# makezur/super_primitive

Measured on AMD Instinct MI355X. Metric: GN iters/sec (640x480x64-seg frame pairs), higher is better.
Workload: dtype f32; 1 GPU; Replica-shaped two-frame SfM, 640x480, 64 segments (grid, 4 px overlap), pyramid level 0 of a 3-level pyramid; BASELINE.json configs[1]; pairs_per_gpu=384, segment_pixels_per_pair=373056, optimiser=gn, tile_points=8192, span_points=4096, granule=64

## Files before the change

### super_primitive_amd/csrc/sp_cost.hip

```cpp
#include <type_traits>

#include "sp_solve_device.h"

namespace {

struct TileCtx {
    gptr_u32 pix;
    gptr_f4 src4;
    gptr_f32 trg;
    Cam Ks;
    Warp w;
    float shift;
    float gain, bias;
    float ax, ay;
    uint32_t row_bytes;
    int Wl, Hl;
    int start, count;
};

struct Geo {
    float qx, qy, qz;
    float zinv, zi;
    float px, py, pz;
};
// ... 293 lines not shown
                                           Pending& p) {
    const f32x2 colrow = rd_colrow(r, lane2);
    const float d = rd_depth(r, DT ? s.w * shift : fast_exp(s.w + shift));
    float x, y;
    backproject(colrow.x, colrow.y, d, c.Ks, ifx, ify, x, y);
    prepare_xyz(c, x, y, d, true, s.x, s.y, s.z, p);
}

__device__ __forceinline__ void prepare2_at(const PairConsts& k, f32x2 colrow, bool src_ok, float d, const f32x4 s, Pending2& p) {
    const f32x2 xy = pfma(colrow, k.ifxy, k.nKc) * d;
    const f32x2 qxy = pfma(k.R03, f32x2{xy.x, xy.x}, pfma(k.R14, f32x2{xy.y, xy.y}, pfma(k.R25, f32x2{d, d}, k.t01)));
    const float qz = fmaf(k.R6, xy.x, fmaf(k.R7, xy.y, fmaf(k.R8, d, k.t2)));
    const bool zguard = fabsf(qz) > 1e-6f;
    const float zinv = zguard ? __builtin_amdgcn_rcpf(qz) : 1e-6f;
    const f32x2 uv = qxy * k.Kf * zinv + k.Ktc;
    const f32x2 n = pfma(uv, k.invWH, f32x2{-1.f, -1.f});
    const bool ok = (fabsf(n.x) <= 0.99f) && (fabsf(n.y) <= 0.99f) && (qz > k.zmin) && src_ok && (d > 1e-7f);
    p.m = ok ? 1.f : 0.f;
    p.qxy = qxy; p.qz = qz;
    p.zinv = ok ? zinv : 0.f;
    p.zi = (ok && zguard) ? zinv : 0.f;
    p.srg = f32x2{s.x, s.y}; p.sb = s.z;
    const f32x2 ixy = pfma(n, k.sxy, k.sxy);
    const f32x2 fl{floorf(ixy.x), floorf(ixy.y)};
    p.wxy = ixy - fl;
    p.off0 = (uint32_t)fmaf(fl.y, k.row_bytes_f, fl.x * (float)(4u * SP_TEXEL_FLOATS));
}

struct Mix2 { f32x2 wa, wb, v; };
struct MixA { f32x2 ua, ub; };
struct AffAcc {
    float haa, hab, hbb, ba, bb;
    f32x2 pa01, pa[2], pb01, pb[2];
    float hda, hdb;
};

template <bool AFF = false>
__device__ __forceinline__ void finish_gn2(const PairConsts& k, const Pending2& p, const f32x3 a, const f32x3 b,
                                           const f32x3 cc, const f32x3 d, Mix2& o, float& cost_acc, float& n_acc,
                                           MixA* oa = nullptr, AffAcc* aa = nullptr) {
    const float eps = k.eps;
    const f32x2 a2{a.x, a.y}, b2{b.x, b.y}, c2{cc.x, cc.y}, d2{d.x, d.y};
    const f32x2 e3 = padd2(psub2(psub2(d2, c2), b2), a2);
    const f32x2 Er{b.x - a.x, cc.x - a.x}, Eg{b.y - a.y, cc.y - a.y}, Eb{b.z - a.z, cc.z - a.z};
    f32x2 e3b;
    e3b.x = (d.z - cc.z) - Eb.x;
    const f32x2 Gr = pfma_swz_lo(p.wxy, e3, Er), Gg = pfma_swz_hi(p.wxy, e3, Eg), Gb = pfma_swz_lo(p.wxy, e3b, Eb);
    const f32x2 it2{fmaf(p.wxy.y, Gr.y, fmaf(p.wxy.x, Er.x, a.x)), fmaf(p.wxy.y, Gg.y, fmaf(p.wxy.x, Eg.x, a.y))};
    const float itb = fmaf(p.wxy.y, Gb.y, fmaf(p.wxy.x, Eb.x, a.z));
    const f32x2 r2 = p.srg - pfma(k.gain, it2, k.bias2);
    const float rb = p.sb - fmaf(k.gain, itb, k.bias2.x);
    const float ar0 = fabsf(r2.x), ar1 = fabsf(r2.y), arb = fabsf(rb);
    auto absmax = [&](float r) { float m; asm("v_max_f32 %0, |%1|, %2" : "=v"(m) : "v"(r), "s"(eps)); return m; };
    const f32x2 wg2{__builtin_amdgcn_rcpf(absmax(r2.x)), __builtin_amdgcn_rcpf(absmax(r2.y))};
    const float wgb = __builtin_amdgcn_rcpf(absmax(rb));
    const f32x2 wGr = pmul_lo(wg2, Gr), wGg = pmul_hi(wg2, Gg), wGb = Gb * wgb;
    o.wa = pfma_lo(wGb, Gb, pfma_lo(wGg, Gg, pmul_lo(wGr, Gr)));
    o.wb = pfma_hi(wGb, Gb, pfma_hi(wGg, Gg, pmul_hi(wGr, Gr)));
    o.v = pfma(wGb, rb, pfma_hi(r2, wGg, pmul_lo(r2, wGr)));
    cost_acc = fmaf(p.m, (ar0 + ar1) + arb, cost_acc);
    n_acc += p.m;
    if constexpr (AFF) {
        const f32x2 ja2 = k.gain * it2;
        const float jab = k.gain * itb;
        const f32x2 wj2 = wg2 * ja2;
        const float wjb = wgb * jab;
        aa->haa = fmaf(p.m, fmaf(wjb, jab, wj2.x * ja2.x) + wj2.y * ja2.y, aa->haa);
        aa->hab = fmaf(-p.m, (wj2.x + wj2.y) + wjb, aa->hab);
        aa->hbb = fmaf(p.m, (wg2.x + wg2.y) + wgb, aa->hbb);
        aa->ba = fmaf(p.m, fmaf(wjb, rb, wj2.x * r2.x) + wj2.y * r2.y, aa->ba);
        aa->bb = fmaf(-p.m, fmaf(wgb, rb, wg2.x * r2.x) + wg2.y * r2.y, aa->bb);
        oa->ua = pfma(Gb, wjb, pfma_hi(wj2, Gg, pmul_lo(wj2, Gr)));
        oa->ub = (wGr + wGg) + wGb;
    }
}

struct GeoGn { f32x2 qxy; float qz, zinv, zi; };
template <bool AFF = false>
__device__ __forceinline__ void fold_gn2(const PairConsts& k, const GeoGn g, const Mix2 w, GnAcc& A, const MixA* wa = nullptr,
                                         AffAcc* aa = nullptr) {
    const f32x2 g2 = k.gab * g.zinv;
    const f32x2 Wa = w.wa * pmul_lo(g2, g2);
    const f32x2 Wb = w.wb * pmul_hi(g2, g2);
    const f32x2 V = -(w.v * g2);
    const f32x2 qxy = g.qxy;
    const f32x2 u = qxy * g.zi;
    const float ez = g.qz - k.t2;
    const f32x2 Q = pfma(-ez, u, qxy - k.t01);
    float nqy;
    asm("v_xor_b32 %0, 0x80000000, %1" : "=v"(nqy) : "v"(qxy.y));
    const f32x2 nA00{u.x, u.x * qxy.y}, A01{fmaf(u.x, qxy.x, g.qz), nqy};
    const f32x2 nA10{u.y, fmaf(u.y, qxy.y, g.qz)}, A11{u.y * qxy.x, qxy.x};
    const f32x2 nB00 = pfma_lo(Wa, nA00, pmul_hi(Wa, nA10)), B01 = pfma_lo(Wa, A01, pmul_hi(Wa, A11));
    const f32x2 nB10 = pfma_lo(Wb, nA00, pmul_hi(Wb, nA10)), B11 = pfma_lo(Wb, A01, pmul_hi(Wb, A11));
    const f32x2 P = pfma_lo(Q, Wa, pmul_hi(Q, Wb));
    A.h00 += Wa; A.h11 += Wb.y;
    A.h0[0] -= nB00; A.h0[1] += B01;
    A.h1[0] -= nB10; A.h1[1] += B11;
    A.blk[0] = pfma_lo(nA00, nB00, pfma_lo(nA10, nB10, A.blk[0]));
    A.blk[1] = pfnma_lo(nA00, B01, pfnma_lo(nA10, B11, A.blk[1]));
    A.blk[2] = pfma_hi(nA00, nB00, pfma_hi(nA10, nB10, A.blk[2]));
    A.blk[3] = pfnma_hi(nA00, B01, pfnma_hi(nA10, B11, A.blk[3]));
    A.blk[4] = pfma_lo(A01, B01, pfma_lo(A11, B11, A.blk[4]));
    A.blk[5] = pfma_hi(A01, B01, pfma_hi(A11, B11, A.blk[5]));
    A.bp01 += V;
    A.hd01 += P;
    A.bp[0] = pfnma_lo(V, nA00, pfnma_hi(V, nA10, A.bp[0]));
    A.bp[1] = pfma_lo(V, A01, pfma_hi(V, A11, A.bp[1]));
    A.hd[0] = pfnma_lo(P, nA00, pfnma_hi(P, nA10, A.hd[0]));
    A.hd[1] = pfma_lo(P, A01, pfma_hi(P, A11, A.hd[1]));
    A.D = pfma(Q, P, A.D);
    A.bd = pfma(Q, V, A.bd);
    if constexpr (AFF) {
        const f32x2 Ua = -(wa->ua * g2), Ub = wa->ub * g2;
        aa->pa01 += Ua;
        aa->pa[0] = pfnma_lo(Ua, nA00, pfnma_hi(Ua, nA10, aa->pa[0]));
        aa->pa[1] = pfma_lo(Ua, A01, pfma_hi(Ua, A11, aa->pa[1]));
        aa->hda = fmaf(Q.x, Ua.x, fmaf(Q.y, Ua.y, aa->hda));
        aa->pb01 += Ub;
        aa->pb[0] = pfnma_lo(Ub, nA00, pfnma_hi(Ub, nA10, aa->pb[0]));
        aa->pb[1] = pfma_lo(Ub, A01, pfma_hi(Ub, A11, aa->pb[1]));
        aa->hdb = fmaf(Q.x, Ub.x, fmaf(Q.y, Ub.y, aa->hdb));
    }
}

typedef const float __attribute__((address_space(4)))* cptr_f32;
struct ChunkRec { int pair, seg, start, count; };
typedef const ChunkRec __attribute__((address_space(4)))* cptr_i4;

struct SpanCursor {
    cptr_i4 chunks;
    cptr_f32 kld, kp_L;
    int q, q_end;
    int left;
    float shift;
    int nq_left;
    float nq_kld, nq_kpl;
};

template <int TRIP = SP_BLOCK>
__device__ __forceinline__ void cursor_fetch_next(SpanCursor& k) {
    if (k.q + 1 < k.q_end) {
        const int seg = k.chunks[k.q + 1].seg;
        k.nq_left = k.chunks[k.q + 1].count / TRIP;
        k.nq_kld = k.kld[seg];
        k.nq_kpl = k.kp_L[seg];
    }
}

template <bool DT>
__device__ __forceinline__ float cursor_shift(float kld, float kpl) { return DT ? fast_exp(kld - kpl) : kld - kpl; }

template <int TRIP = SP_BLOCK, bool DT = false>
__device__ __forceinline__ void cursor_init(SpanCursor& k, const SpPair& pr, const int4* chunks, int q0, int n) {
    k.chunks = (cptr_i4)chunks;
    k.kld = (cptr_f32)pr.kld;
    k.kp_L = (cptr_f32)pr.kp_L;
    k.q = q0; k.q_end = q0 + n;
    const int seg0 = k.chunks[q0].seg;
    k.left = k.chunks[q0].count / TRIP;
    k.shift = cursor_shift<DT>(k.kld[seg0], k.kp_L[seg0]);
    k.nq_left = 0; k.nq_kld = 0.f; k.nq_kpl = 0.f;
    cursor_fetch_next<TRIP>(k);
}

template <int TRIP = SP_BLOCK, bool DT = false>
__device__ __forceinline__ bool cursor_advance(SpanCursor& k, int& done_q) {
    done_q = k.q;
    if (--k.left > 0) return false;
    ++k.q;
    k.left = k.nq_left;
    k.shift = cursor_shift<DT>(k.nq_kld, k.nq_kpl);
    cursor_fetch_next<TRIP>(k);
    return true;
}

template <bool WT>
__device__ __forceinline__ void store_partial(float* p, float v) {
    if (WT) __hip_atomic_store(p, v, __ATOMIC_RELAXED, __HIP_MEMORY_SCOPE_AGENT);
    else *p = v;
}

__device__ __forceinline__ int lane_id() { return (int)__builtin_amdgcn_mbcnt_hi(~0u, __builtin_amdgcn_mbcnt_lo(~0u, 0u)); }

template <bool WT, bool AFF = false>
__device__ __forceinline__ void flush_segment_gn(GnAcc& A, float* __restrict__ rec, AffAcc* aa = nullptr) {
    const int lane = lane_id();
    int pos; bool ok;
    if constexpr (AFF) {
        float v[10] = {A.hd01.x, A.hd01.y, A.hd[0].x, A.hd[0].y, A.hd[1].x, A.hd[1].y, A.D.x + A.D.y, A.bd.x + A.bd.y, aa->hda, aa->hdb};
        wave_sum_to_lanes<10>(v, lane, pos, ok);
        if (ok) store_partial<WT>(rec + pos, v[0]);
        aa->hda = 0.f; aa->hdb = 0.f;
    } else {
        float v[10] = {A.hd01.x, A.hd01.y, A.hd[0].x, A.hd[0].y, A.hd[1].x, A.hd[1].y, A.D.x + A.D.y, A.bd.x + A.bd.y,
                       A.cost - A.cost_mark, A.n - A.n_mark};
        wave_sum_to_lanes<10>(v, lane, pos, ok);
        if (ok) store_partial<WT>(rec + pos, v[0]);
        A.cost_mark = A.cost; A.n_mark = A.n;
    }
    const f32x2 z{0.f, 0.f};
    A.hd01 = z; A.hd[0] = z; A.hd[1] = z; A.D = z; A.bd = z;
}

template <bool DT, bool WT, bool AFF = false, bool W64 = false, bool RD = false>
__device__ __forceinline__ void run_span_gn(const TileCtx& c, const SpPair& pr, const int4* __restrict__ chunks, int q0,
                                            int n_chunks, int total, float irls_eps, float* __restrict__ span_rec,
                                            float* __restrict__ seg_partials, float* lds, const SpRunDesc* rd = nullptr) {
    static_assert(!RD || (W64 && DT && !AFF), "run descriptors: wave spans on depth tables");
    constexpr int TRIP = W64 ? 64 : SP_BLOCK;
    constexpr int NV = AFF ? SP_GNA_PARTIAL_FLOATS : SP_GN_PARTIAL_FLOATS, NS = AFF ? SP_GNA_SEG_FLOATS : SP_GN_SEG_FLOATS;
    GnAcc A;
    AffAcc AA;
    MixA ma{f32x2{0.f, 0.f}, f32x2{0.f, 0.f}};
    {
        const f32x2 z{0.f, 0.f};
        AA.haa = AA.hab = AA.hbb = AA.ba = AA.bb = AA.hda = AA.hdb = 0.f;
        AA.pa01 = z; AA.pb01 = z; AA.pa[0] = z; AA.pa[1] = z; AA.pb[0] = z; AA.pb[1] = z;
    }
    {
        const f32x2 z{0.f, 0.f};
        A.h00 = z; A.bp01 = z; A.hd01 = z;
#pragma unroll
        for (int k = 0; k < 2; ++k) { A.h0[k] = z; A.h1[k] = z; A.bp[k] = z; A.hd[k] = z; }
#pragma unroll
        for (int k = 0; k < 6; ++k) A.blk[k] = z;
        A.D = z; A.bd = z;
        A.h11 = A.cost = A.n = A.cost_mark = A.n_mark = 0.f;
    }
    const int wave = __builtin_amdgcn_readfirstlane((int)(threadIdx.x >> 6));
    SpanCursor k;
    cursor_init<TRIP, DT>(k, pr, chunks, q0, n_chunks);
    const int start = k.chunks[q0].start;
    PairConsts kc;
    {
        const Warp& w = c.w;
        kc.ifxy = sgpr2(1.f / c.Ks.fx, 1.f / c.Ks.fy);
        kc.nKc = f32x2{-c.Ks.cx * (1.f / c.Ks.fx), -c.Ks.cy * (1.f / c.Ks.fy)};
        kc.R03 = sgpr2(w.R[0], w.R[3]);        kc.R14 = sgpr2(w.R[1], w.R[4]);      kc.R25 = sgpr2(w.R[2], w.R[5]);
        kc.t01 = f32x2{w.t[0], w.t[1]};        kc.Kf = sgpr2(w.Kt.fx, w.Kt.fy);     kc.Ktc = sgpr2(w.Kt.cx, w.Kt.cy);
        kc.invWH = sgpr2(2.f * w.invWm1, 2.f * w.invHm1);  kc.sxy = sgpr2(w.sx, w.sy);
        kc.gab = sgpr2(c.gain * c.ax * w.Kt.fx, c.gain * c.ay * w.Kt.fy);
        kc.bias2 = f32x2{c.bias, c.bias};      kc.eps2 = sgpr2(irls_eps, irls_eps);
        kc.R6 = sgpr(w.R[6]); kc.R7 = sgpr(w.R[7]); kc.R8 = sgpr(w.R[8]); kc.t2 = w.t[2];
        asm volatile("" : "+v"(kc.nKc), "+v"(kc.bias2), "+v"(kc.t01), "+v"(kc.t2));
        kc.gain = sgpr(c.gain); kc.bias = sgpr(c.bias); kc.zmin = sgpr(w.zmin); kc.eps = sgpr(irls_eps);
        kc.row_bytes_f = sgpr((float)(c.Wl * (int)(4u * SP_TEXEL_FLOATS)));
    }
    const rsrc_t r_pix = make_rsrc(c.pix + start, (uint32_t)total * 4u);
    const rsrc_t r_src = make_rsrc(c.src4 + start, (uint32_t)total * 16u);
    const rsrc_t r_trg = make_rsrc(c.trg, (uint32_t)c.Wl * (uint32_t)c.Hl * (4u * SP_TEXEL_FLOATS));
    const int n_iter = total / TRIP;
    uint32_t op = (W64 ? (threadIdx.x & 63u) : threadIdx.x) * 4u;
    constexpr int NT = 2;
    cptr_rd rg = (cptr_rd)rd + (start >> 6);
    f32x2 lane2{(float)(threadIdx.x & 63u), 0.f};
    if (RD) asm volatile("" : "+v"(lane2));
    struct Slot { Pending2 p; int q; bool last; };
    Slot S0, S1;
    {
        const f32x4 s = buf_load4<NT>(r_src, op * 4u);
        if (RD) prepare2_rd<DT>(kc, k.shift, rd_load(rg), lane2, s, S0.p);
        else {
            const uint32_t pw = (uint32_t)__builtin_amdgcn_raw_buffer_load_b32(r_pix, (int)op, 0, NT);
            prepare2<DT>(c, kc, k.shift, pw, s, S0.p);
        }
        S0.last = cursor_advance<TRIP, DT>(k, S0.q);
    }
    S1.p = S0.p;
    S1.p.zinv = 0.f; S1.p.zi = 0.f;
    S1.q = q0; S1.last = false;
    Mix2 m{f32x2{0.f, 0.f}, f32x2{0.f, 0.f}, f32x2{0.f, 0.f}};
    auto trip = [&](Slot& a, Slot& b) {
        op += 4u * TRIP;
        asm volatile("" : "+v"(op));
        const uint32_t pw = RD ? 0u : (uint32_t)__builtin_amdgcn_raw_buffer_load_b32(r_pix, (int)op, 0, NT);
        const f32x4 s = buf_load4<NT>(r_src, op * 4u);
        SpRunDesc rn;
        if (RD) { ++rg; rn = rd_load(rg); }
        f32x3 ta = buf_load3(r_trg, a.p.off0);
        f32x3 tb = buf_load3(r_trg, a.p.off0 + 4u * SP_TEXEL_FLOATS);
        f32x3 tc = buf_load3(r_trg, a.p.off0, c.row_bytes);
        f32x3 td = buf_load3(r_trg, a.p.off0 + 4u * SP_TEXEL_FLOATS, c.row_bytes);
        __builtin_amdgcn_sched_barrier(0);
        fold_gn2<AFF>(kc, GeoGn{b.p.qxy, b.p.qz, b.p.zinv, b.p.zi}, m, A, &ma, &AA);
        if (b.last) flush_segment_gn<WT, AFF>(A, seg_partials + (size_t)(W64 ? b.q : 4 * b.q + wave) * NS, &AA);
        __builtin_amdgcn_sched_barrier(0);
        asm volatile("" : "+v"(ta), "+v"(tb), "+v"(tc), "+v"(td), "+v"(A.blk[0]), "+v"(A.blk[1]), "+v"(A.blk[2]),
                     "+v"(A.blk[3]), "+v"(A.blk[4]), "+v"(A.blk[5]), "+v"(A.bp[0]), "+v"(A.bp[1]), "+v"(A.hd[0]),
                     "+v"(A.hd[1]), "+v"(A.D), "+v"(A.bd), "+v"(A.h00), "+v"(A.h0[0]), "+v"(A.h0[1]), "+v"(A.h1[0]), "+v"(A.h1[1]), "+v"(A.h11), "+v"(A.bp01), "+v"(A.hd01));
        finish_gn2<AFF>(kc, a.p, ta, tb, tc, td, m, A.cost, A.n, &ma, &AA);
        uint32_t pw_ = pw;
        f32x4 s_ = s;
        if (RD) asm volatile("" : "+v"(s_));
        else asm volatile("" : "+v"(pw_), "+v"(s_));
        if (RD) prepare2_rd<DT>(kc, k.shift, rn, lane2, s_, b.p);
        else prepare2<DT>(c, kc, k.shift, pw_, s_, b.p);
        b.last = cursor_advance<TRIP, DT>(k, b.q);
    };
    int j = 0;
    for (; j + 1 < n_iter; j += 2) { trip(S0, S1); trip(S1, S0); }
    if (j < n_iter) {
        trip(S0, S1);
        fold_gn2<AFF>(kc, GeoGn{S0.p.qxy, S0.p.qz, S0.p.zinv, S0.p.zi}, m, A, &ma, &AA);
        flush_segment_gn<WT, AFF>(A, seg_partials + (size_t)(W64 ? S0.q : 4 * S0.q + wave) * NS, &AA);
    } else {
        fold_gn2<AFF>(kc, GeoGn{S1.p.qxy, S1.p.qz, S1.p.zinv, S1.p.zi}, m, A, &ma, &AA);
        flush_segment_gn<WT, AFF>(A, seg_partials + (size_t)(W64 ? S1.q : 4 * S1.q + wave) * NS, &AA);
    }
    float acc[NV];
    acc[0] = A.cost;
    acc[1] = A.h00.x; acc[2] = A.h00.y;
    acc[3] = A.h0[0].x; acc[4] = A.h0[0].y; acc[5] = A.h0[1].x; acc[6] = A.h0[1].y;
    acc[7] = A.h11;
    acc[8] = A.h1[0].x; acc[9] = A.h1[0].y; acc[10] = A.h1[1].x; acc[11] = A.h1[1].y;
    acc[12] = A.blk[0].x; acc[13] = A.blk[0].y; acc[14] = A.blk[1].x; acc[15] = A.blk[1].y;
    acc[16] = A.blk[2].y; acc[17] = A.blk[3].x; acc[18] = A.blk[3].y;
    acc[19] = A.blk[4].x; acc[20] = A.blk[4].y; acc[21] = A.blk[5].y;
    acc[22] = A.bp01.x; acc[23] = A.bp01.y;
    acc[24] = A.bp[0].x; acc[25] = A.bp[0].y; acc[26] = A.bp[1].x; acc[27] = A.bp[1].y;
    acc[28] = A.n;
    if constexpr (AFF) {
        acc[29] = AA.haa; acc[30] = AA.hab; acc[31] = AA.hbb; acc[32] = AA.ba; acc[33] = AA.bb;
        acc[34] = AA.pa01.x; acc[35] = AA.pa01.y; acc[36] = AA.pa[0].x; acc[37] = AA.pa[0].y; acc[38] = AA.pa[1].x; acc[39] = AA.pa[1].y;
        acc[40] = AA.pb01.x; acc[41] = AA.pb01.y; acc[42] = AA.pb[0].x; acc[43] = AA.pb[0].y; acc[44] = AA.pb[1].x; acc[45] = AA.pb[1].y;
        acc[46] = acc[47] = 0.f;
    } else {
        acc[29] = acc[30] = acc[31] = 0.f;
    }
    if (W64) {
        int pos; bool ok;
        wave_sum_to_lanes<NV>(acc, (int)((op >> 2) & 63u), pos, ok);
        if (ok) store_partial<WT>(span_rec + pos, acc[0]);
    } else {
        const int tid = (int)((op >> 2) & (uint32_t)(SP_BLOCK - 1));
        const float tot = block_sum_to_thread<NV>(acc, lds, tid);
        if (tid < NV) store_partial<WT>(span_rec + tid, tot);
    }
}

template <bool DT, bool WT, bool W64 = false, bool RD = false>
__device__ __forceinline__ void run_span_grad(const TileCtx& c, const SpPair& pr, const int4* __restrict__ chunks, int q0,
                                              int n_chunks, int total, float* __restrict__ span_rec,
                                              float* __restrict__ seg_partials, float* lds, const SpRunDesc* rd = nullptr) {
    static_assert(!RD || (W64 && DT), "run descriptors: wave spans on depth tables");
    constexpr int TRIP = W64 ? 64 : SP_BLOCK;
    constexpr int NV = SP_GRAD_PARTIAL_FLOATS;
    float acc[NV];
#pragma unroll
    for (int i = 0; i < NV; ++i) acc[i] = 0.f;
    const int wave = __builtin_amdgcn_readfirstlane((int)(threadIdx.x >> 6));
    SpanCursor k;
    cursor_init<TRIP, DT>(k, pr, chunks, q0, n_chunks);
    const int start = k.chunks[q0].start;
    const float ifx = 1.f / c.Ks.fx, ify = 1.f / c.Ks.fy;
    const rsrc_t r_pix = make_rsrc(c.pix + start, (uint32_t)total * 4u);
    const rsrc_t r_src = make_rsrc(c.src4 + start, (uint32_t)total * 16u);
    const rsrc_t r_trg = make_rsrc(c.trg, (uint32_t)c.Wl * (uint32_t)c.Hl * (4u * SP_TEXEL_FLOATS));
    const int n_iter = total / TRIP;
    uint32_t op = (W64 ? (threadIdx.x & 63u) : threadIdx.x) * 4u;
    constexpr int NT = 2;
    cptr_rd rg = (cptr_rd)rd + (start >> 6);
    f32x2 lane2{(float)(threadIdx.x & 63u), 0.f};
    if (RD) asm volatile("" : "+v"(lane2));
    struct Slot { Pending p; int q; bool last; };
    Slot S0, S1;
    {
        const f32x4 s = buf_load4<NT>(r_src, op * 4u);
        if (RD) prepare_rd<DT>(c, k.shift, ifx, ify, rd_load(rg), lane2, s, S0.p);
        else {
            const uint32_t pw = (uint32_t)__builtin_amdgcn_raw_buffer_load_b32(r_pix, (int)op, 0, NT);
            prepare<DT>(c, k.shift, ifx, ify, pw, s, S0.p);
        }
        S0.last = cursor_advance<TRIP, DT>(k, S0.q);
    }
    S1.p = S0.p;
    S1.p.g.zinv = 0.f; S1.p.g.zi = 0.f;
    S1.q = q0; S1.last = false;
    Mix0 m0{0.f, 0.f, 0.f, 0.f};
    auto flush = [&](int q) {
        const float tot = wave_sum(acc[13]);
        if (lane_id() == 0) store_partial<WT>(seg_partials + (size_t)(W64 ? q : 4 * q + wave) * SP_GRAD_SEG_FLOATS, tot);
        acc[13] = 0.f;
    };
    auto trip = [&](Slot& a, Slot& b) {
        op += 4u * TRIP;
        asm volatile("" : "+v"(op));
        const uint32_t pw = RD ? 0u : (uint32_t)__builtin_amdgcn_raw_buffer_load_b32(r_pix, (int)op, 0, NT);
        const f32x4 s = buf_load4<NT>(r_src, op * 4u);
        SpRunDesc rn;
        if (RD) { ++rg; rn = rd_load(rg); }
        f32x3 ta = buf_load3(r_trg, a.p.off0);
        f32x3 tb = buf_load3(r_trg, a.p.off0 + 4u * SP_TEXEL_FLOATS);
        f32x3 tc = buf_load3(r_trg, a.p.off0, c.row_bytes);
        f32x3 td = buf_load3(r_trg, a.p.off0 + 4u * SP_TEXEL_FLOATS, c.row_bytes);
        __builtin_amdgcn_sched_barrier(0);
        fold_grad(c, b.p.g, m0, acc);
        if (b.last) flush(b.q);
        __builtin_amdgcn_sched_barrier(0);
        asm volatile("" : "+v"(ta), "+v"(tb), "+v"(tc), "+v"(td), "+v"(acc[1]), "+v"(acc[2]), "+v"(acc[3]), "+v"(acc[4]), "+v"(acc[5]),
                     "+v"(acc[6]), "+v"(acc[7]), "+v"(acc[8]), "+v"(acc[9]), "+v"(acc[10]), "+v"(acc[11]), "+v"(acc[12]),
                     "+v"(acc[13]), "+v"(acc[14]), "+v"(acc[15]));
        finish_grad(c, a.p, ta, tb, tc, td, m0, acc[0]);
        uint32_t pw_ = pw;
        f32x4 s_ = s;
        if (RD) asm volatile("" : "+v"(s_));
        else asm volatile("" : "+v"(pw_), "+v"(s_));
        if (RD) prepare_rd<DT>(c, k.shift, ifx, ify, rn, lane2, s_, b.p);
        else prepare<DT>(c, k.shift, ifx, ify, pw_, s_, b.p);
        b.last = cursor_advance<TRIP, DT>(k, b.q);
    };
    int j = 0;
    for (; j + 1 < n_iter; j += 2) { trip(S0, S1); trip(S1, S0); }
    if (j < n_iter) {
        trip(S0, S1);
        fold_grad(c, S0.p.g, m0, acc);
        flush(S0.q);
    } else {
        fold_grad(c, S1.p.g, m0, acc);
        flush(S1.q);
    }
    if (W64) {
        int pos; bool ok;
        wave_sum_to_lanes<NV>(acc, (int)((op >> 2) & 63u), pos, ok);
        if (ok) store_partial<WT>(span_rec + pos, acc[0]);
    } else {
        const int tid = (int)((op >> 2) & (uint32_t)(SP_BLOCK - 1));
        const float tot = block_sum_to_thread<NV>(acc, lds, tid);
        if (tid < NV) store_partial<WT>(span_rec + tid, tot);
    }
}

__device__ __forceinline__ void fill_warp(TileCtx& c, const float* pose, const Cam& Kt, int H, int W, int Hl, int Wl,
                                          float zmin) {
    load_pose(pose, c.w.R, c.w.t);
    c.w.Kt = Kt;
    c.w.invWm1 = sgpr(1.f / (float)(W - 1));
    c.w.invHm1 = sgpr(1.f / (float)(H - 1));
    c.w.sx = sgpr(0.5f * (float)(Wl - 1));
    c.w.sy = sgpr(0.5f * (float)(Hl - 1));
    c.w.zmin = zmin;
    c.Wl = Wl; c.Hl = Hl;
    c.row_bytes = (uint32_t)Wl * (4u * SP_TEXEL_FLOATS);
    c.ax = sgpr(2.f * c.w.sx * c.w.invWm1);
    c.ay = sgpr(2.f * c.w.sy * c.w.invHm1);
}


struct SingleArgs {
    const uint32_t* pix; const float4* src4; const float* kp_L; const int4* tiles;
    const float* K_src; const float* kld; const float* trg; const float* K_trg; const float* pose;
    const float* aff_src; const float* aff_trg;
    int n_tiles, H, W, Hl, Wl;
    float zmin;
};

__global__ __launch_bounds__(SP_BLOCK) void k_cost_single_grad(SingleArgs a, float* __restrict__ partials) {
    __shared__ float lds[SP_WAVES * SP_GRAD_PARTIAL_FLOATS];
    const int t = xcd_chunked_tile(blockIdx.x, a.n_tiles);
    if (t >= a.n_tiles) return;
    const int b = blockIdx.y;
    const int4 tile = a.tiles[t];
    TileCtx c;
    c.pix = (gptr_u32)a.pix; c.src4 = (gptr_f4)a.src4;
    c.trg = (gptr_f32)(a.trg + (size_t)b * a.Hl * a.Wl * SP_TEXEL_FLOATS);
    load_cam(a.K_src, c.Ks);
    Cam Kt; load_cam(a.K_trg + 9 * b, Kt);
    fill_warp(c, a.pose + 16 * b, Kt, a.H, a.W, a.Hl, a.Wl, a.zmin);
    c.shift = a.kld[tile.y] - a.kp_L[tile.y];
    c.gain = 1.f; c.bias = 0.f;
    if (a.aff_src) {
        c.gain = expf(-(a.aff_trg[2 * b] - a.aff_src[0]));
        c.bias = a.aff_trg[2 * b + 1] - a.aff_src[1];
    }
    c.start = tile.z; c.count = tile.w;
    run_tile<false>(c, partials + ((size_t)b * a.n_tiles + t) * SP_GRAD_PARTIAL_FLOATS, lds);
}

#define SP_POINT_TILE 2048
struct PointsArgs {
    const float* xyz; const float* rgb; const float* trg; const float* K_trg; const float* pose;
    const float* aff_src; const float* aff_trg;
    int n_points, n_tiles, H, W, Hl, Wl;
    float zmin;
};

__global__ __launch_bounds__(SP_BLOCK) void k_cost_points_grad(PointsArgs a, float* __restrict__ partials) {
    __shared__ float lds[SP_WAVES * SP_GRAD_PARTIAL_FLOATS];
    const int t = xcd_chunked_tile(blockIdx.x, a.n_tiles);
    if (t >= a.n_tiles) return;
    const int b = blockIdx.y;
    TileCtx c;
    c.pix = (gptr_u32)a.xyz; c.src4 = (gptr_f4)a.rgb;
    c.trg = (gptr_f32)(a.trg + (size_t)b * a.Hl * a.Wl * SP_TEXEL_FLOATS);
    c.Ks = Cam{1.f, 1.f, 0.f, 0.f};
    Cam Kt; load_cam(a.K_trg + 9 * b, Kt);
    fill_warp(c, a.pose + 16 * b, Kt, a.H, a.W, a.Hl, a.Wl, a.zmin);
    c.shift = 0.f;
    c.gain = 1.f; c.bias = 0.f;
    if (a.aff_src) {
        c.gain = expf(-(a.aff_trg[2 * b] - a.aff_src[0]));
        c.bias = a.aff_trg[2 * b + 1] - a.aff_src[1];
    }
    c.start = t * SP_POINT_TILE;
    c.count = min(SP_POINT_TILE, a.n_points - c.start);
    run_tile<true>(c, partials + ((size_t)b * a.n_tiles + t) * SP_GRAD_PARTIAL_FLOATS, lds);
}

__global__ __launch_bounds__(SP_BLOCK) void k_finalise_single(const float* __restrict__ partials,
                                                               const int32_t* __restrict__ seg_tile_off, int n_tiles,
                                                               int N, int P, bool has_aff, float* residual,
                                                               float* g_kld, float* g_pose, float* g_aff) {
    const int b = blockIdx.x;
    const float* p = partials + (size_t)b * n_tiles * SP_GRAD_PARTIAL_FLOATS;
    const double scale = 1.0 / (3.0 * (double)P);
    const int lane = threadIdx.x & 63, wave = threadIdx.x >> 6;
    for (int k = wave; k < SP_GRAD_PARTIAL_FLOATS; k += SP_WAVES) {
        if (k == 13) continue;
        double s = 0.0;
        for (int t = lane; t < n_tiles; t += 64) s += (double)p[(size_t)t * SP_GRAD_PARTIAL_FLOATS + k];
#pragma unroll
        for (int o = 32; o > 0; o >>= 1) s += __shfl_xor(s, o, 64);
        if (lane == 0) {
            const float v = (float)(s * scale);
            if (k == 0) residual[b] = v;
            else if (k <= 3) g_pose[b * 16 + (k - 1) * 4 + 3] = v;
            else if (k <= 12) { const int e = k - 4; g_pose[b * 16 + (e / 3) * 4 + (e % 3)] = v; }
            else if (k == 14) { g_aff[b * 4 + 2] = has_aff ? v : 0.f; g_aff[b * 4 + 0] = has_aff ? -v : 0.f; }
            else { g_aff[b * 4 + 3] = has_aff ? v : 0.f; g_aff[b * 4 + 1] = has_aff ? -v : 0.f; }
        }
    }
    if (threadIdx.x < 4) g_pose[b * 16 + 12 + threadIdx.x] = 0.f;
    for (int n = threadIdx.x; n < N; n += SP_BLOCK) {
        double s = 0.0;
        for (int t = seg_tile_off[n]; t < seg_tile_off[n + 1]; ++t) s += (double)p[(size_t)t * SP_GRAD_PARTIAL_FLOATS + 13];
        g_kld[(size_t)b * N + n] = (float)(s * scale);
    }
}

#define SP_SCHED_LISTS 8
struct SchedList {
    const int4* chunks;
    const int4* spans;
    float* partials;
    float* seg_partials;
    int32_t n_spans;
    int32_t first_block;
    uint32_t mask;
    int32_t vspans;
};
struct SchedCost {
    const SpPair* pairs[SP_MAX_PHASES];
    float irls_eps[SP_MAX_PHASES];
    uint32_t mask;
    int32_t vspans;
    int32_t n_lists;
    SchedList list[SP_SCHED_LISTS];
};
struct FuseArgs {
    int32_t* arrivals;
    AdamArgs adam;
    GnArgs gn;
    const int32_t* done;
    const int32_t* phase;
    SchedCost sched;
    const int32_t* active;
    const MultiList* multi;
    int32_t n_multi;
    const uint32_t* rd_pix;
    const SpRunDesc* rd_desc;
};

constexpr int FORM_LOG_DEPTH = 0, FORM_DEPTH = 6;
// ... 419 lines not shown
```

### super_primitive_amd/csrc/sp_device.h

```cpp
#pragma once
#include <hip/hip_runtime.h>
#include <stdint.h>
#include "../../include/sp_hip.h"

#define SP_BLOCK 256
#define SP_WAVES (SP_BLOCK / 64)

typedef const uint32_t __attribute__((address_space(1)))* gptr_u32;
typedef float f32x4 __attribute__((ext_vector_type(4)));
typedef const f32x4 __attribute__((address_space(1)))* gptr_f4;
typedef const float __attribute__((address_space(1)))* gptr_f32;

__device__ __forceinline__ float4 ntload4(gptr_f4 p) {
    const f32x4 v = __builtin_nontemporal_load(p);
    return make_float4(v.x, v.y, v.z, v.w);
}

__device__ __forceinline__ float fast_exp(float x) {
    const float log2e_hi = 1.44269502162933349609375f, log2e_lo = 1.92596299112661746e-8f;
    const float hi = x * log2e_hi;
    const float lo = fmaf(x, log2e_hi, -hi) + x * log2e_lo;
    return __builtin_amdgcn_exp2f(hi) * (1.0f + 0.693147180559945f * lo);
}

#define SP_CHECK_LAUNCH()                          \
    do {                                           \
        hipError_t e__ = hipGetLastError();        \
        if (e__ != hipSuccess) return (int)e__;    \
    } while (0)
static inline int sp_hip_rc(hipError_t e) { return e == hipSuccess ? 0 : -(1000 + (int)e); }

struct SpSchedule;
struct SpQueue;
struct MultiList {
    const SpPair* pairs;
    const int32_t* chunks;
    const int32_t* spans;
    float* partials;
    float* seg_partials;
    int32_t n_spans;
    int32_t first_block;
};
__attribute__((visibility("hidden"))) int cost_pairs_multi(const MultiList* lists_dev, int n_lists, int total_blocks, int mode, float irls_eps, void* stream);

struct ChainImgJob { const float* in; float* out; float* packed; };
__attribute__((visibility("hidden"))) int chain_pyramid_multi(const ChainImgJob* jobs_dev, int n, int n_levels, int H, int W, void* stream);
struct ChainComposeJob { const SpPair* pairs; const SpWindowEdge* edges; SpWindowNode* nodes; int32_t n_edges, n_nodes; };
__attribute__((visibility("hidden"))) int chain_compose_multi(const ChainComposeJob* jobs_dev, int n, void* stream);
__attribute__((visibility("hidden"))) int chain_compose_max_edges(void);
struct ChainCritJob {
    const uint32_t* pix; const float* baseL; const int32_t* seg_off; const float* kp_L; const float* kld; const float* K;
    const float* rel_pose; const float* pose; const float* kf_pose;
    unsigned long long* keys; float* depth; uint32_t* ws; float* crit;
    int32_t N, P;
};
__attribute__((visibility("hidden"))) int chain_criterion_multi(const ChainCritJob* jobs_dev, int n, int max_P, int H, int W, float thresh, void* stream);
struct WgnMultiInfo { int total_blocks, max_edges, max_blocks, max_y, n_reduce; };
__attribute__((visibility("hidden"))) int wgn_multi_args_bytes(void);
__attribute__((visibility("hidden"))) int wgn_multi_fill(const SpWindowGn* const* windows, int n, int flags, float lm_up, float lm_down, float lm_min,
                                                          float conv_tol, bool allow_inline, void* args_host, MultiList* lists_host, WgnMultiInfo* info);
__attribute__((visibility("hidden"))) int wgn_multi_round(const void* args_dev, const MultiList* lists_dev, int n, const WgnMultiInfo& info, int flags,
                                                           float irls_eps, void* stream);
__attribute__((visibility("hidden"))) int wgn_multi_gather(const void* args_dev, int n, float* out, void* stream);
struct ScheduleCostFrom {
    int first_phase;
    const SpQueue* queue;
    int n_slots;
    const int32_t* active;
    int n_active;
    uint32_t idle_mask;
};
__attribute__((visibility("hidden"))) int schedule_cost_from(const SpSchedule* sched, const int32_t* phase, void* stream, const ScheduleCostFrom& from);

__device__ __forceinline__ float wave_sum(float v) {
#pragma unroll
    for (int o = 32; o > 0; o >>= 1) v += __shfl_xor(v, o, 64);
    return v;
}

template <int N, int OFF, class T>
__device__ __forceinline__ void halve_step(T* v, bool upper) {
    constexpr int H = (N + 1) / 2;
#pragma unroll
    for (int k = 0; k < H; ++k) {
        const T lo = v[k];
        const T hi = (k + H < N) ? v[k + H] : T(0);
        const T keep = upper ? hi : lo;
        const T give = upper ? lo : hi;
        v[k] = keep + __shfl_xor(give, OFF, 64);
    }
}

template <int NV, class T>
__device__ __forceinline__ void wave_sum_to_lanes(T (&acc)[NV], int lane, int& pos, bool& ok) {
    static_assert(NV <= 64, "one value per lane at most");
    constexpr int N0 = NV, N1 = (N0 + 1) / 2, N2 = (N1 + 1) / 2, N3 = (N2 + 1) / 2, N4 = (N3 + 1) / 2, N5 = (N4 + 1) / 2;
    halve_step<N0, 32>(acc, lane & 32);
    halve_step<N1, 16>(acc, lane & 16);
    halve_step<N2, 8>(acc, lane & 8);
    halve_step<N3, 4>(acc, lane & 4);
    halve_step<N4, 2>(acc, lane & 2);
    halve_step<N5, 1>(acc, lane & 1);
    pos = 0;
    ok = true;
    if (lane & 1)  { pos += (N5 + 1) / 2; ok = ok && pos < N5; }
    if (lane & 2)  { pos += (N4 + 1) / 2; ok = ok && pos < N4; }
    if (lane & 4)  { pos += (N3 + 1) / 2; ok = ok && pos < N3; }
    if (lane & 8)  { pos += (N2 + 1) / 2; ok = ok && pos < N2; }
    if (lane & 16) { pos += (N1 + 1) / 2; ok = ok && pos < N1; }
    if (lane & 32) { pos += (N0 + 1) / 2; ok = ok && pos < N0; }
}

template <int NV>
__device__ __forceinline__ float block_sum_to_thread(float (&acc)[NV], float* lds , int tid) {
    const int lane = tid & 63, wave = tid >> 6;
    int pos;
    bool ok;
    wave_sum_to_lanes<NV>(acc, lane, pos, ok);
    if (ok) lds[wave * NV + pos] = acc[0];
    __syncthreads();
    float total = 0.f;
    if (tid < NV) {
#pragma unroll
        for (int w = 0; w < SP_WAVES; ++w) total += lds[w * NV + tid];
    }
    return total;
}
template <int NV>
__device__ __forceinline__ float block_sum_to_thread(float (&acc)[NV], float* lds) {
    return block_sum_to_thread<NV>(acc, lds, (int)threadIdx.x);
}

__device__ __forceinline__ int xcd_chunked_tile(int b, int n) {
    const int per = (n + 7) >> 3;
    const int t = (b & 7) * per + (b >> 3);
    return t;
}

struct Cam {
    float fx, fy, cx, cy;
};

struct PointGeom {
    float px, py, pz;
    float qx, qy, qz;
    float zinv;
    bool  zguard;
    float ix, iy;
    bool  valid;
};

__device__ __forceinline__ void decode_pix(uint32_t w, float& col, float& row, bool& src_ok) {
    col = (float)(w & 0xffffu);
    row = (float)((w >> 16) & 0x7fffu);
    src_ok = (w >> 31) != 0u;
}

__device__ __forceinline__ void backproject(float col, float row, float d, const Cam& K, float ifx, float ify,
                                            float& x, float& y) {
    x = ((col - K.cx) * d) * ifx;
    y = ((row - K.cy) * d) * ify;
}

struct Warp {
    float R[9], t[3];
    Cam Kt;
    float invWm1, invHm1;
    float sx, sy;
    float zmin;
};

__device__ __forceinline__ void warp_point(const Warp& w, float px, float py, float pz, PointGeom& g) {
    g.px = px; g.py = py; g.pz = pz;
    g.qx = fmaf(w.R[0], px, fmaf(w.R[1], py, w.R[2] * pz)) + w.t[0];
    g.qy = fmaf(w.R[3], px, fmaf(w.R[4], py, w.R[5] * pz)) + w.t[1];
    g.qz = fmaf(w.R[6], px, fmaf(w.R[7], py, w.R[8] * pz)) + w.t[2];
    g.zguard = fabsf(g.qz) > 1e-6f;
    g.zinv = g.zguard ? __builtin_amdgcn_rcpf(g.qz) : 1e-6f;
    const float u = g.qx * w.Kt.fx * g.zinv + w.Kt.cx;
    const float v = g.qy * w.Kt.fy * g.zinv + w.Kt.cy;
    const float xn = 2.f * u * w.invWm1 - 1.f;
    const float yn = 2.f * v * w.invHm1 - 1.f;
    g.valid = (fabsf(xn) <= 0.99f) && (fabsf(yn) <= 0.99f) && (g.qz > w.zmin);
    g.ix = (xn + 1.f) * w.sx;
    g.iy = (yn + 1.f) * w.sy;
}

#define SP_TEXEL_FLOATS 3

struct Taps {
    float4 t00, t10, t01, t11;
    float wx, wy;
};

__device__ __forceinline__ void fetch_taps(gptr_f32 img, int Wl, int Hl, float ix, float iy, Taps& tp) {
    const float fx0 = floorf(ix), fy0 = floorf(iy);
    tp.wx = ix - fx0;
    tp.wy = iy - fy0;
    const int x0 = (int)fx0, y0 = (int)fy0;
    const int x1 = x0 + 1, y1 = y0 + 1;
    const bool inx0 = (x0 >= 0) & (x0 < Wl), inx1 = (x1 >= 0) & (x1 < Wl);
    const bool iny0 = (y0 >= 0) & (y0 < Hl), iny1 = (y1 >= 0) & (y1 < Hl);
    const int cx0 = min(max(x0, 0), Wl - 1), cx1 = min(max(x1, 0), Wl - 1);
    const int cy0 = min(max(y0, 0), Hl - 1), cy1 = min(max(y1, 0), Hl - 1);
    struct Rgb { float x, y, z; };
    auto texel = [&](int yy, int xx) { gptr_f32 q = img + (size_t)(yy * Wl + xx) * SP_TEXEL_FLOATS; return Rgb{q[0], q[1], q[2]}; };
    const Rgb a = texel(cy0, cx0), b = texel(cy0, cx1);
    const Rgb c = texel(cy1, cx0), d = texel(cy1, cx1);
    const float m00 = (inx0 & iny0) ? 1.f : 0.f, m10 = (inx1 & iny0) ? 1.f : 0.f;
    const float m01 = (inx0 & iny1) ? 1.f : 0.f, m11 = (inx1 & iny1) ? 1.f : 0.f;
    tp.t00 = make_float4(a.x * m00, a.y * m00, a.z * m00, 0.f);
    tp.t10 = make_float4(b.x * m10, b.y * m10, b.z * m10, 0.f);
    tp.t01 = make_float4(c.x * m01, c.y * m01, c.z * m01, 0.f);
    tp.t11 = make_float4(d.x * m11, d.y * m11, d.z * m11, 0.f);
}

__device__ __forceinline__ float bilerp(float a00, float a10, float a01, float a11, float wx, float wy) {
    const float top = fmaf(wx, a10 - a00, a00);
    const float bot = fmaf(wx, a11 - a01, a01);
    return fmaf(wy, bot - top, top);
}

__device__ __forceinline__ float sgn(float v) { return (v > 0.f) ? 1.f : ((v < 0.f) ? -1.f : 0.f); }

__device__ __forceinline__ void load_cam(const float* __restrict__ K9, Cam& c) {
    c.fx = K9[0]; c.cx = K9[2]; c.fy = K9[4]; c.cy = K9[5];
}

__device__ __forceinline__ void load_pose(const float* __restrict__ T16, float (&R)[9], float (&t)[3]) {
    R[0] = T16[0]; R[1] = T16[1]; R[2] = T16[2];  t[0] = T16[3];
    R[3] = T16[4]; R[4] = T16[5]; R[5] = T16[6];  t[1] = T16[7];
    R[6] = T16[8]; R[7] = T16[9]; R[8] = T16[10]; t[2] = T16[11];
}
```

Measured before the change: 453,800 iters/s.

## Use permlane swaps and DPP for wave reductions; peel first pipeline trip

The halving wave reduction for float accumulators now uses permlane32/permlane16 swap instructions for the wide strides and DPP row moves for the narrow strides, in place of ds_bpermute-based shuffles. This is meant to cut LDS-path latency and instruction count in the per-segment and end-of-block reductions. Separately, the first software-pipeline trip is peeled with a compile-time flag, so the dummy fold on a zeroed slot and the slot-copy initialisation are dropped. The risk is correctness of the hand-chosen DPP control codes and permlane semantics, which apply only to gfx950-class hardware.

After: 456,200 iters/s (median of 6 runs). No clear change (+0.5%).

```diff
diff --git a/super_primitive_amd/csrc/sp_cost.hip b/super_primitive_amd/csrc/sp_cost.hip
--- a/super_primitive_amd/csrc/sp_cost.hip
+++ b/super_primitive_amd/csrc/sp_cost.hip
@@ -469,16 +469,17 @@
 __device__ __forceinline__ float cursor_shift(float kld, float kpl) { return DT ? fast_exp(kld - kpl) : kld - kpl; }
 
 template <int TRIP = SP_BLOCK, bool DT = false>
-__device__ __forceinline__ void cursor_init(SpanCursor& k, const SpPair& pr, const int4* chunks, int q0, int n) {
+__device__ __forceinline__ int cursor_init(SpanCursor& k, const SpPair& pr, const int4* chunks, int q0, int n) {
     k.chunks = (cptr_i4)chunks;
     k.kld = (cptr_f32)pr.kld;
     k.kp_L = (cptr_f32)pr.kp_L;
     k.q = q0; k.q_end = q0 + n;
-    const int seg0 = k.chunks[q0].seg;
+    const int seg0 = k.chunks[q0].seg, start = k.chunks[q0].start;
     k.left = k.chunks[q0].count / TRIP;
     k.shift = cursor_shift<DT>(k.kld[seg0], k.kp_L[seg0]);
     k.nq_left = 0; k.nq_kld = 0.f; k.nq_kpl = 0.f;
     cursor_fetch_next<TRIP>(k);
+    return start;
 }
 
 template <int TRIP = SP_BLOCK, bool DT = false>
@@ -547,8 +548,7 @@
     }
     const int wave = __builtin_amdgcn_readfirstlane((int)(threadIdx.x >> 6));
     SpanCursor k;
-    cursor_init<TRIP, DT>(k, pr, chunks, q0, n_chunks);
-    const int start = k.chunks[q0].start;
+    const int start = cursor_init<TRIP, DT>(k, pr, chunks, q0, n_chunks);
     PairConsts kc;
     {
         const Warp& w = c.w;
@@ -584,11 +584,8 @@
         }
         S0.last = cursor_advance<TRIP, DT>(k, S0.q);
     }
-    S1.p = S0.p;
-    S1.p.zinv = 0.f; S1.p.zi = 0.f;
-    S1.q = q0; S1.last = false;
-    Mix2 m{f32x2{0.f, 0.f}, f32x2{0.f, 0.f}, f32x2{0.f, 0.f}};
-    auto trip = [&](Slot& a, Slot& b) {
+    Mix2 m;
+    auto trip = [&](Slot& a, Slot& b, auto first) {
         op += 4u * TRIP;
         asm volatile("" : "+v"(op));
         const uint32_t pw = RD ? 0u : (uint32_t)__builtin_amdgcn_raw_buffer_load_b32(r_pix, (int)op, 0, NT);
@@ -600,8 +597,10 @@
         f32x3 tc = buf_load3(r_trg, a.p.off0, c.row_bytes);
         f32x3 td = buf_load3(r_trg, a.p.off0 + 4u * SP_TEXEL_FLOATS, c.row_bytes);
         __builtin_amdgcn_sched_barrier(0);
-        fold_gn2<AFF>(kc, GeoGn{b.p.qxy, b.p.qz, b.p.zinv, b.p.zi}, m, A, &ma, &AA);
-        if (b.last) flush_segment_gn<WT, AFF>(A, seg_partials + (size_t)(W64 ? b.q : 4 * b.q + wave) * NS, &AA);
+        if constexpr (!decltype(first)::value) {
+            fold_gn2<AFF>(kc, GeoGn{b.p.qxy, b.p.qz, b.p.zinv, b.p.zi}, m, A, &ma, &AA);
+            if (b.last) flush_segment_gn<WT, AFF>(A, seg_partials + (size_t)(W64 ? b.q : 4 * b.q + wave) * NS, &AA);
+        }
         __builtin_amdgcn_sched_barrier(0);
         asm volatile("" : "+v"(ta), "+v"(tb), "+v"(tc), "+v"(td), "+v"(A.blk[0]), "+v"(A.blk[1]), "+v"(A.blk[2]),
                      "+v"(A.blk[3]), "+v"(A.blk[4]), "+v"(A.blk[5]), "+v"(A.bp[0]), "+v"(A.bp[1]), "+v"(A.hd[0]),
@@ -615,15 +614,16 @@
         else prepare2<DT>(c, kc, k.shift, pw_, s_, b.p);
         b.last = cursor_advance<TRIP, DT>(k, b.q);
     };
-    int j = 0;
-    for (; j + 1 < n_iter; j += 2) { trip(S0, S1); trip(S1, S0); }
+    trip(S0, S1, std::true_type{});
+    int j = 1;
+    for (; j + 1 < n_iter; j += 2) { trip(S1, S0, std::false_type{}); trip(S0, S1, std::false_type{}); }
     if (j < n_iter) {
-        trip(S0, S1);
+        trip(S1, S0, std::false_type{});
+        fold_gn2<AFF>(kc, GeoGn{S1.p.qxy, S1.p.qz, S1.p.zinv, S1.p.zi}, m, A, &ma, &AA);
+        flush_segment_gn<WT, AFF>(A, seg_partials + (size_t)(W64 ? S1.q : 4 * S1.q + wave) * NS, &AA);
+    } else {
         fold_gn2<AFF>(kc, GeoGn{S0.p.qxy, S0.p.qz, S0.p.zinv, S0.p.zi}, m, A, &ma, &AA);
         flush_segment_gn<WT, AFF>(A, seg_partials + (size_t)(W64 ? S0.q : 4 * S0.q + wave) * NS, &AA);
-    } else {
-        fold_gn2<AFF>(kc, GeoGn{S1.p.qxy, S1.p.qz, S1.p.zinv, S1.p.zi}, m, A, &ma, &AA);
-        flush_segment_gn<WT, AFF>(A, seg_partials + (size_t)(W64 ? S1.q : 4 * S1.q + wave) * NS, &AA);
     }
     float acc[NV];
     acc[0] = A.cost;
@@ -668,8 +668,7 @@
     for (int i = 0; i < NV; ++i) acc[i] = 0.f;
     const int wave = __builtin_amdgcn_readfirstlane((int)(threadIdx.x >> 6));
     SpanCursor k;
-    cursor_init<TRIP, DT>(k, pr, chunks, q0, n_chunks);
-    const int start = k.chunks[q0].start;
+    const int start = cursor_init<TRIP, DT>(k, pr, chunks, q0, n_chunks);
     const float ifx = 1.f / c.Ks.fx, ify = 1.f / c.Ks.fy;
     const rsrc_t r_pix = make_rsrc(c.pix + start, (uint32_t)total * 4u);
     const rsrc_t r_src = make_rsrc(c.src4 + start, (uint32_t)total * 16u);
@@ -691,16 +690,13 @@
         }
         S0.last = cursor_advance<TRIP, DT>(k, S0.q);
     }
-    S1.p = S0.p;
-    S1.p.g.zinv = 0.f; S1.p.g.zi = 0.f;
-    S1.q = q0; S1.last = false;
-    Mix0 m0{0.f, 0.f, 0.f, 0.f};
+    Mix0 m0;
     auto flush = [&](int q) {
         const float tot = wave_sum(acc[13]);
         if (lane_id() == 0) store_partial<WT>(seg_partials + (size_t)(W64 ? q : 4 * q + wave) * SP_GRAD_SEG_FLOATS, tot);
         acc[13] = 0.f;
     };
-    auto trip = [&](Slot& a, Slot& b) {
+    auto trip = [&](Slot& a, Slot& b, auto first) {
         op += 4u * TRIP;
         asm volatile("" : "+v"(op));
         const uint32_t pw = RD ? 0u : (uint32_t)__builtin_amdgcn_raw_buffer_load_b32(r_pix, (int)op, 0, NT);
@@ -712,8 +708,10 @@
         f32x3 tc = buf_load3(r_trg, a.p.off0, c.row_bytes);
         f32x3 td = buf_load3(r_trg, a.p.off0 + 4u * SP_TEXEL_FLOATS, c.row_bytes);
         __builtin_amdgcn_sched_barrier(0);
-        fold_grad(c, b.p.g, m0, acc);
-        if (b.last) flush(b.q);
+        if constexpr (!decltype(first)::value) {
+            fold_grad(c, b.p.g, m0, acc);
+            if (b.last) flush(b.q);
+        }
         __builtin_amdgcn_sched_barrier(0);
         asm volatile("" : "+v"(ta), "+v"(tb), "+v"(tc), "+v"(td), "+v"(acc[1]), "+v"(acc[2]), "+v"(acc[3]), "+v"(acc[4]), "+v"(acc[5]),
                      "+v"(acc[6]), "+v"(acc[7]), "+v"(acc[8]), "+v"(acc[9]), "+v"(acc[10]), "+v"(acc[11]), "+v"(acc[12]),
@@ -727,15 +725,16 @@
         else prepare<DT>(c, k.shift, ifx, ify, pw_, s_, b.p);
         b.last = cursor_advance<TRIP, DT>(k, b.q);
     };
-    int j = 0;
-    for (; j + 1 < n_iter; j += 2) { trip(S0, S1); trip(S1, S0); }
+    trip(S0, S1, std::true_type{});
+    int j = 1;
+    for (; j + 1 < n_iter; j += 2) { trip(S1, S0, std::false_type{}); trip(S0, S1, std::false_type{}); }
     if (j < n_iter) {
-        trip(S0, S1);
+        trip(S1, S0, std::false_type{});
+        fold_grad(c, S1.p.g, m0, acc);
+        flush(S1.q);
+    } else {
         fold_grad(c, S0.p.g, m0, acc);
         flush(S0.q);
-    } else {
-        fold_grad(c, S1.p.g, m0, acc);
-        flush(S1.q);
     }
     if (W64) {
         int pos; bool ok;
diff --git a/super_primitive_amd/csrc/sp_device.h b/super_primitive_amd/csrc/sp_device.h
--- a/super_primitive_amd/csrc/sp_device.h
+++ b/super_primitive_amd/csrc/sp_device.h
@@ -78,29 +78,48 @@
     return v;
 }
 
-template <int N, int OFF, class T>
+template <int CTRL>
+__device__ __forceinline__ float dpp_f32(float v) {
+    return __builtin_bit_cast(float, __builtin_amdgcn_update_dpp(0, __builtin_bit_cast(int, v), CTRL, 0xf, 0xf, true));
+}
+template <int N, int OFF, bool XLANE, class T>
 __device__ __forceinline__ void halve_step(T* v, bool upper) {
     constexpr int H = (N + 1) / 2;
 #pragma unroll
     for (int k = 0; k < H; ++k) {
         const T lo = v[k];
         const T hi = (k + H < N) ? v[k + H] : T(0);
-        const T keep = upper ? hi : lo;
-        const T give = upper ? lo : hi;
-        v[k] = keep + __shfl_xor(give, OFF, 64);
+        if constexpr (!XLANE) {
+            const T keep = upper ? hi : lo;
+            const T give = upper ? lo : hi;
+            v[k] = keep + __shfl_xor(give, OFF, 64);
+        } else if constexpr (OFF >= 16) {
+            const uint32_t a = __builtin_bit_cast(uint32_t, lo), b = __builtin_bit_cast(uint32_t, hi);
+            const auto r = OFF == 32 ? __builtin_amdgcn_permlane32_swap(a, b, false, false) : __builtin_amdgcn_permlane16_swap(a, b, false, false);
+            const uint32_t mine = r[0], theirs = r[1];
+            v[k] = __builtin_bit_cast(float, mine) + __builtin_bit_cast(float, theirs);
+        } else {
+            constexpr int FROM_ABOVE = OFF == 8 ? 0x128 : OFF == 4 ? 0x12C : OFF == 2 ? 0x4E : 0xB1;
+            constexpr int FROM_BELOW = OFF == 8 ? 0x128 : OFF == 4 ? 0x124 : OFF == 2 ? 0x4E : 0xB1;
+            const float s_lo = lo + dpp_f32<FROM_ABOVE>(lo);
+            float s_hi = 0.f;
+            if (k + H < N) s_hi = hi + dpp_f32<FROM_BELOW>(hi);
+            v[k] = upper ? s_hi : s_lo;
+        }
     }
 }
 
-template <int NV, class T>
+template <int NV, class T, bool XLANE = __is_same(T, float)>
 __device__ __forceinline__ void wave_sum_to_lanes(T (&acc)[NV], int lane, int& pos, bool& ok) {
     static_assert(NV <= 64, "one value per lane at most");
+    static_assert(!XLANE || __is_same(T, float), "the swap / DPP exchanges are written for floats");
     constexpr int N0 = NV, N1 = (N0 + 1) / 2, N2 = (N1 + 1) / 2, N3 = (N2 + 1) / 2, N4 = (N3 + 1) / 2, N5 = (N4 + 1) / 2;
-    halve_step<N0, 32>(acc, lane & 32);
-    halve_step<N1, 16>(acc, lane & 16);
-    halve_step<N2, 8>(acc, lane & 8);
-    halve_step<N3, 4>(acc, lane & 4);
-    halve_step<N4, 2>(acc, lane & 2);
-    halve_step<N5, 1>(acc, lane & 1);
+    halve_step<N0, 32, XLANE>(acc, lane & 32);
+    halve_step<N1, 16, XLANE>(acc, lane & 16);
+    halve_step<N2, 8, XLANE>(acc, lane & 8);
+    halve_step<N3, 4, XLANE>(acc, lane & 4);
+    halve_step<N4, 2, XLANE>(acc, lane & 2);
+    halve_step<N5, 1, XLANE>(acc, lane & 1);
     pos = 0;
     ok = true;
     if (lane & 1)  { pos += (N5 + 1) / 2; ok = ok && pos < N5; }
```
